# ingra14m/RobIR

Measured on AMD Instinct MI355X. Metric: PBR-stage rays/sec (128 SG lobes, 32 visibility samples/lobe), full forward render, higher is better.
Workload: dtype f32 (every MLP -- light visibility, SDF values and reverse-mode gradient, colour, visibility, 512-wide and CESR nets: every fp32 operand exact as three f16 pieces, six MFMA products per multiply-add in three fp32 accumulators -- in the light-visibility kernel the two outer products of the 2^-22 clas

## Files before the change

robir_amd/csrc/vis_diffuse_x6t.hip:

```cpp
#include "../../include/robir_hip.h"
#include "common.h"
#include "mlp_engine.h"
#include "x6_ring.h"

namespace rb {

#define RB_TINY 1e-6f
constexpr int XT_MAX_DIRS = 4096;
constexpr int XT_WF4 = 1536;
constexpr int XT_CF4 = 4 + XT_WF4;
constexpr int XT_SLOTS = 4, XT_DIST = 3;
constexpr int XT_PIECES = 6;
#ifndef XT_FP8
#define XT_FP8 1
#endif
template <int N>
struct XtInt {
  static constexpr int value = N;
};
__host__ __device__ constexpr bool xt_slot_tile0(int s) { return s == 0 || s == 1 || (s >= 4 && s <= 7); }

__device__ __forceinline__ void xt_dma16(const f4* gbase_uniform, unsigned lane_byte_off, unsigned lds_byte_uniform) {
  asm volatile("s_mov_b32 m0, %0\n\ts_nop 0\n\tglobal_load_lds_dwordx4 %1, %2" ::"s"(lds_byte_uniform), "v"(lane_byte_off),
               "s"(gbase_uniform)
               : "memory");
}
template <int OFF>
__device__ __forceinline__ void xt_dma16_imm(const f4* gbase_uniform, unsigned lane_byte_off, unsigned lds_byte_uniform) {
  asm volatile("s_mov_b32 m0, %0\n\ts_nop 0\n\tglobal_load_lds_dwordx4 %1, %2 offset:%3" ::"s"(lds_byte_uniform), "v"(lane_byte_off),
               "s"(gbase_uniform), "n"(OFF)
               : "memory");
}

template <int OFF>
__device__ __forceinline__ void xt_dma16_m0kept(const f4* gbase_uniform, unsigned lane_byte_off) {
  asm volatile("global_load_lds_dwordx4 %0, %1 offset:%2" ::"v"(lane_byte_off), "s"(gbase_uniform), "n"(OFF) : "memory");
}

struct XtTile {
  int point;
  int dir_base;
};
struct XtArgs {
  const float *A, *Bd;
  const f4* W49;
  int argmax_vis;
  unsigned* range_word;
  const float *normals, *dirs, *wdir, *wsum;
  const int* cid;
  int L, nsamp;
  float* vis_out;
  unsigned long long* eval_count;
  const unsigned short* pair_j;
  const XtTile* tile_info;
  const unsigned long long* counters;
  float* pair_vis;
};

template <bool STREAM>
__global__ __launch_bounds__(256, 1) void k_dvis_x6t(const XtArgs a) {
  __shared__ f4 ring[XT_SLOTS * XT_WF4];
  __shared__ f4 headw[XT_WF4];
  __shared__ f4 bias_tab[49 * 4];
  __shared__ f4 aux[(XT_MAX_DIRS * 4 + XT_MAX_DIRS * 2) / 16 + 64];
  __shared__ int s_count;
  float* const vis_tab = reinterpret_cast<float*>(aux);
  unsigned short* const idx_list = reinterpret_cast<unsigned short*>(aux + XT_MAX_DIRS / 4);
  f4* const a_row = aux + (XT_MAX_DIRS * 6) / 16;
  f4* const a_rows = aux;
  const float* __restrict__ A = a.A;
  const float* __restrict__ Bd = a.Bd;
  const f4* __restrict__ W49 = a.W49;
  const int argmax_vis = a.argmax_vis;
  const int tid = threadIdx.x, lane = tid & 63, g = lane >> 4;
  const int wave = __builtin_amdgcn_readfirstlane(tid >> 6);
  const float negk = -2048.0f;
  constexpr float C11 = 1.0f / 2048.0f;
  const long p = blockIdx.x;
  const int L = a.L, nsamp = a.nsamp, LS = L * nsamp;
  long dbase = 0;
  int S = 0, rounds = 0;
  const int G = gridDim.x;
  long total_tiles = 0, total_rounds = 0;
  for (int i = tid; i < 49 * 4; i += 256) bias_tab[i] = W49[(long)(i >> 2) * XT_CF4 + (i & 3)];
  for (int i = tid; i < XT_WF4; i += 256) headw[i] = W49[48L * XT_CF4 + 4 + i];
  if constexpr (STREAM) {
    total_tiles = (long)a.counters[0];
    total_rounds = (total_tiles + 7) >> 3;
    __syncthreads();
    if ((long)blockIdx.x >= total_rounds) return;
    rounds = 1;
  } else {
  const float* __restrict__ normals = a.normals;
  const float* __restrict__ dirs = a.dirs;
  const int* __restrict__ cid = a.cid;
  dbase = (cid ? (long)cid[p] : 0L) * LS;
  if (tid == 0) s_count = 0;
  if (tid < 64) a_row[tid] = reinterpret_cast<const f4*>(A + p * 256)[tid];
  for (int j = tid; j < LS; j += 256) vis_tab[j] = 0.f;
  __syncthreads();
  const float nx = normals[3 * p], ny = normals[3 * p + 1], nz = normals[3 * p + 2];
  for (int j0 = 0; j0 < LS; j0 += 256) {
    const int j = j0 + tid;
    bool front = false;
    if (j < LS) {
      const float* d = dirs + 3 * (dbase + j);
      const float c = nx * d[0] + ny * d[1] + nz * d[2];
      front = c > RB_TINY;
    }
    const unsigned long long mk = __ballot(front);
    int base = 0;
    if (lane == 0 && mk) base = atomicAdd(&s_count, __popcll(mk));
    base = __shfl(base, 0);
    if (front) idx_list[base + __popcll(mk & ((1ull << lane) - 1ull))] = (unsigned short)j;
  }
  __syncthreads();
  S = s_count;
  if (tid == 0 && a.eval_count) atomicAdd(a.eval_count, (unsigned long long)S);
  rounds = (S + 127) / 128;
  }

  const unsigned ring_b = (unsigned)(unsigned long)((__attribute__((address_space(3))) char*)ring);
  unsigned voff_a = (unsigned)wave * 6144u + (unsigned)lane * 16u, voff_b = voff_a + 4096u;
  asm volatile("" : "+v"(voff_a), "+v"(voff_b));
  const unsigned wave_lds = ring_b + (unsigned)wave * 6144u;
  typedef const __attribute__((address_space(3))) u4* lds_u4p;
  unsigned ring_a0 = ring_b + (unsigned)lane * 16u, ring_a2 = ring_a0 + 2u * XT_WF4 * 16u;
  asm volatile("" : "+v"(ring_a0), "+v"(ring_a2));
  const lds_u4p ring_u = (lds_u4p)ring_a0, ring_u2 = (lds_u4p)ring_a2;
  u4 wh[4], wm[4], wl[4];
#if XT_FP8
  typedef int xt_i8 __attribute__((ext_vector_type(8)));
  xt_i8 w8h, w8l;
#define XT_F16OFF(KB, PIECE) (((KB) >> 2) * 768 + (((KB) & 3) * 2 + (PIECE)) * 64)
#define XT_LOAD8(DST, BASE, OFF)                                                                                             \
  {                                                                                                                          \
    const u4 a_ = (BASE)[(OFF)], b_ = (BASE)[(OFF) + 64];                                                                    \
    DST = xt_i8{(int)a_[0], (int)a_[1], (int)a_[2], (int)a_[3], (int)b_[0], (int)b_[1], (int)b_[2], (int)b_[3]};             \
  }
#endif
  f4 bias;
  if (rounds > 0) {
#pragma unroll
    for (int c = 0; c < 3; ++c)
#pragma unroll
      for (int i = 0; i < XT_PIECES; ++i)
        xt_dma16(W49 + (long)c * XT_CF4 + 4 + i * 64, voff_a, wave_lds + (unsigned)c * 24576u + (unsigned)i * 1024u);
    asm volatile("s_waitcnt vmcnt(12)" ::: "memory");
    __builtin_amdgcn_s_barrier();
    asm volatile("" ::: "memory");
#pragma unroll
    for (int k = 0; k < 4; ++k) {
#if XT_FP8
      wh[k] = ring_u[XT_F16OFF(k, 0)];
      wm[k] = ring_u[XT_F16OFF(k, 1)];
#else
      wh[k] = ring_u[(k * 3 + 0) * 64];
      wm[k] = ring_u[(k * 3 + 1) * 64];
      wl[k] = ring_u[(k * 3 + 2) * 64];
#endif
    }
#if XT_FP8
    XT_LOAD8(w8h, ring_u, 512)
    XT_LOAD8(w8l, ring_u, 640)
#endif
    bias = bias_tab[g];
  }

  unsigned sat = 0u;
#if XT_FP8
  struct Ops {
    u4 h[2][8], m[2][8];
    xt_i8 h8[2][2], l8[2][2];
  };
  unsigned el_keep[2] = {0u, 0u};
#else
  struct Ops {
    u4 h[2][8], m[2][8], l[2][8];
  };
#endif
  Ops P, Q;

#define XT_MFMA(ACC, WREG, XREG) \
  ACC = __builtin_amdgcn_mfma_f32_16x16x32_f16(__builtin_bit_cast(h8, WREG), __builtin_bit_cast(h8, XREG), ACC, 0, 0, 0)

  float ev0[2][2], ev1[2][2], ed0, ed1;
  unsigned eh;
  SxAcc prev[2];
  auto ep_stage1 = [&](int t, int q) {
    const SxAcc& a = prev[t];
    const float r0 = __builtin_fmaf(__builtin_fmaf(a.c2[2 * q], C11, a.c1[2 * q]), C11, a.c0[2 * q]);
    const float r1 = __builtin_fmaf(__builtin_fmaf(a.c2[2 * q + 1], C11, a.c1[2 * q + 1]), C11, a.c0[2 * q + 1]);
    ev0[t][q] = fmaxf(r0, 0.f);
    ev1[t][q] = fmaxf(r1, 0.f);
  };
  auto ep_stage2 = [&](int t, int q) {
    const unsigned hu = __builtin_bit_cast(unsigned, __builtin_amdgcn_cvt_pkrtz(ev0[t][q], ev1[t][q]));
    const float s0 = ev0[t][q] * 2048.0f, s1 = ev1[t][q] * 2048.0f;
    asm("v_fma_mix_f32 %0, %1, %2, %3 op_sel_hi:[1,0,0]" : "=v"(ed0) : "v"(hu), "s"(negk), "v"(s0));
    asm("v_fma_mix_f32 %0, %1, %2, %3 op_sel:[1,0,0] op_sel_hi:[1,0,0]" : "=v"(ed1) : "v"(hu), "s"(negk), "v"(s1));
    eh = hu;
    sat = sat_acc_nonneg(sat, hu);
  };
  auto ep_stage3 = [&](Ops& Y, int t, int jb, int q) {
    const unsigned mu = __builtin_bit_cast(unsigned, __builtin_amdgcn_cvt_pkrtz(ed0, ed1));
    const float e0 = ed0 * 2048.0f, e1 = ed1 * 2048.0f;
    unsigned lu;
    asm("v_fma_mixlo_f16 %0, %1, %2, %3 op_sel_hi:[1,0,0]" : "=v"(lu) : "v"(mu), "s"(negk), "v"(e0));
    asm("v_fma_mixhi_f16 %0, %1, %2, %3 op_sel:[1,0,0] op_sel_hi:[1,0,0]" : "+v"(lu) : "v"(mu), "s"(negk), "v"(e1));
    Y.h[t][jb >> 1][(jb & 1) * 2 + q] = eh;
    Y.m[t][jb >> 1][(jb & 1) * 2 + q] = mu;
#if XT_FP8
    if (q == 0) {
      el_keep[t] = lu;
    } else {
      Y.h8[t][jb >> 3][jb & 7] = (int)__builtin_amdgcn_perm(eh, Y.h[t][jb >> 1][(jb & 1) * 2], 0x07050301u);
      Y.l8[t][jb >> 3][jb & 7] = (int)__builtin_amdgcn_perm(lu, el_keep[t], 0x07050301u);
    }
#else
    Y.l[t][jb >> 1][(jb & 1) * 2 + q] = lu;
#endif
  };
  auto ep_slot = [&](Ops& Y, int s, int pj) {
    switch (s) {
      case 0: ep_stage1(0, 0); break;
      case 1: ep_stage1(0, 1); break;
      case 2: ep_stage1(1, 0); break;
      case 3: ep_stage1(1, 1); break;
      case 4: ep_stage2(0, 0); break;
      case 5: ep_stage3(Y, 0, pj, 0); break;
      case 6: ep_stage2(0, 1); break;
      case 7: ep_stage3(Y, 0, pj, 1); break;
      case 8: ep_stage2(1, 0); break;
      case 9: ep_stage3(Y, 1, pj, 0); break;
      case 10: ep_stage2(1, 1); break;
      default: ep_stage3(Y, 1, pj, 1); break;
    }
  };

  f4 raw[2][16];
  int jj[2], jjn[2];
  int tpn[2] = {-1, -1}, tbn[2] = {0, 0}, jn2[2] = {0xFFFF, 0xFFFF};
  const unsigned arow_b = (unsigned)(unsigned long)((__attribute__((address_space(3))) char*)a_rows);
  XtTile recn[2] = {{-1, 0}, {-1, 0}};
  bool okn[2] = {false, false};
  auto tile_lookup = [&](long round) {
#pragma unroll
    for (int t = 0; t < 2; ++t) {
      const long T = round * 8 + wave * 2 + t;
      okn[t] = round < total_rounds && T < total_tiles;
      const long Tc = T < total_tiles ? T : total_tiles - 1;
      recn[t] = a.tile_info[Tc];
      jn2[t] = (int)a.pair_j[Tc * 16 + (lane & 15)];
    }
  };
  auto tile_resolve = [&]() {
#pragma unroll
    for (int t = 0; t < 2; ++t) {
      tpn[t] = okn[t] ? __builtin_amdgcn_readfirstlane(recn[t].point) : -1;
      tbn[t] = okn[t] ? __builtin_amdgcn_readfirstlane(recn[t].dir_base) : 0;
      if (!okn[t]) jn2[t] = 0xFFFF;
    }
  };
  auto fetch_rows = [&](long rd_next, int parity_next) {
    if constexpr (STREAM) {
      tile_resolve();
#pragma unroll
      for (int t = 0; t < 2; ++t) {
        const long prow = tpn[t] < 0 ? 0L : (long)tpn[t];
        xt_dma16(reinterpret_cast<const f4*>(A + prow * 256), (unsigned)lane * 16u,
                 arow_b + (unsigned)(parity_next * 8 + wave * 2 + t) * 1024u);
      }
    }
#pragma unroll
    for (int t = 0; t < 2; ++t) {
      long row;
      if constexpr (STREAM) {
        jjn[t] = (tpn[t] < 0 || jn2[t] == 0xFFFF) ? -1 : jn2[t];
        row = (long)tbn[t] + (jjn[t] < 0 ? 0 : jjn[t]);
      } else {
        const int si = (int)rd_next * 128 + t * 64 + wave * 16 + (lane & 15);
        jjn[t] = si < S ? (int)idx_list[si] : -1;
        row = dbase + (jjn[t] < 0 ? 0 : jjn[t]);
      }
      const f4* brow = reinterpret_cast<const f4*>(Bd + row * 256) + g;
#pragma unroll
      for (int kb = 0; kb < 16; ++kb) raw[t][kb] = brow[kb * 4];
    }
  };
  long rd = STREAM ? (long)blockIdx.x : 0L;
  const long rd_end = STREAM ? total_rounds : (long)rounds, rd_step = STREAM ? (long)G : 1L;
  int parity = 0;
  if constexpr (STREAM) tile_lookup(rd);
  if (rounds > 0) fetch_rows(rd, 0);
#ifdef XT_TIMING
#define XT_T(i) { const unsigned long long t_ = __builtin_amdgcn_s_memtime(); tacc[i] += t_ - tlast; tlast = t_; }
  unsigned long long tacc[4] = {0, 0, 0, 0}, tlast = __builtin_amdgcn_s_memtime();
  int trounds = 0;
#else
#define XT_T(i)
#endif
  {
    auto round_body = [&](auto ntc) __attribute__((always_inline)) {
    constexpr int NT = decltype(ntc)::value;
#pragma unroll
    for (int t = 0; t < NT; ++t) {
      jj[t] = jjn[t];
      const f4* arow = STREAM ? a_rows + (parity * 8 + wave * 2 + t) * 64 : a_row;
#pragma unroll
      for (int kb = 0; kb < 16; ++kb) {
        const f4 bv = raw[t][kb];
        const f4 av = arow[kb * 4 + g];
#pragma unroll
        for (int q = 0; q < 2; ++q) {
          unsigned h, m, l;
          sx_split_pair(fmaxf(av[2 * q] + bv[2 * q], 0.f), fmaxf(av[2 * q + 1] + bv[2 * q + 1], 0.f), negk, h, m, l);
          P.h[t][kb / 2][(kb & 1) * 2 + q] = h;
          P.m[t][kb / 2][(kb & 1) * 2 + q] = m;
#if XT_FP8
          if (q == 0) {
            el_keep[t] = l;
          } else {
            P.h8[t][kb >> 3][kb & 7] = (int)__builtin_amdgcn_perm(h, P.h[t][kb / 2][(kb & 1) * 2], 0x07050301u);
            P.l8[t][kb >> 3][kb & 7] = (int)__builtin_amdgcn_perm(l, el_keep[t], 0x07050301u);
          }
#else
          P.l[t][kb / 2][(kb & 1) * 2 + q] = l;
#endif
          sat = sat_acc_nonneg(sat, h);
        }
      }
    }
    XT_T(0)
    auto layer = [&](int l, Ops& X, Ops& Y) __attribute__((always_inline)) {
      const f4* Wl = W49 + (long)l * 16 * XT_CF4 + 4;
      const f4* Wn = W49 + (long)(l == 2 ? 0 : l + 1) * 16 * XT_CF4 + 4;
#pragma unroll
      for (int jb = 0; jb < 16; ++jb) {
        SxAcc acc[2];
        asm volatile("s_waitcnt vmcnt(6)" ::: "memory");
#ifndef XT_ABL_NOBAR
        __builtin_amdgcn_s_barrier();
#endif
        asm volatile("" ::: "memory");
        const int nx3 = jb + XT_DIST;
        const f4* dsrc = nx3 < 16 ? Wl + (long)nx3 * XT_CF4 : Wn + (long)(nx3 - 16) * XT_CF4;
        const unsigned ddst = wave_lds + (unsigned)(nx3 & 3) * 24576u;
        const f4 nbias = bias_tab[(l * 16 + jb + 1) * 4 + g];
#if defined(XT_ABL_NODMA)
#define XT_COPY(I) do { } while (0)
#else
#define XT_COPY(I)                                                                  \
  do {                                                                              \
    if ((I) == 0) xt_dma16_imm<0>(dsrc, voff_a, ddst);                              \
    else if ((I) < 4) xt_dma16_m0kept<((I) & 3) * 1024>(dsrc, voff_a);              \
    else if ((I) == 4) xt_dma16_imm<0>(dsrc, voff_b, ddst + 4096u);                 \
    else xt_dma16_m0kept<((I) & 3) * 1024>(dsrc, voff_b);                           \
  } while (0)
#endif
#define XT_FENCE __builtin_amdgcn_sched_barrier(0)
#ifdef XT_ABL_NOLDS
#define XT_FRAG(DST, KB, PIECE) asm volatile("" : "+v"(DST))
#else
#if XT_FP8
#define XT_FRAG(DST, KB, PIECE) DST = nfrag[XT_F16OFF(KB, PIECE)]
#else
#define XT_FRAG(DST, KB, PIECE) DST = nfrag[((KB) * 3 + (PIECE)) * 64]
#endif
#endif
#define XT_MFMA8(ACC, WREG, XREG) ACC = __builtin_amdgcn_mfma_scale_f32_16x16x128_f8f6f4(WREG, XREG, ACC, 1, 1, 0, 0, 0, 0)
#define XT_EP(S)                        \
  do {                                  \
    if (jb > 0) ep_slot(Y, (S), jb - 1); \
  } while (0)
#define XT_RUN(ACC, WP, XP)                     \
  _Pragma("unroll") for (int k_ = 0; k_ < 4; ++k_) { \
    const int k = H ? 3 - k_ : k_;               \
    XT_MFMA(ACC, WP[k], XP[4 * H + k]);          \
  }
#define XT_RUN_REFILL(ACC, WP, XP, PIECE)          \
  _Pragma("unroll") for (int k_ = 0; k_ < 4; ++k_) { \
    const int k = H ? 3 - k_ : k_;                   \
    XT_MFMA(ACC, WP[k], XP[4 * H + k]);              \
// ... 128 lines not shown
#if !XT_FP8
          P.l[t][kb] = Q.l[t][kb];
#endif
        }
#if XT_FP8
#pragma unroll
      for (int t = 0; t < NT; ++t)
#pragma unroll
        for (int hf = 0; hf < 2; ++hf) {
          P.h8[t][hf] = Q.h8[t][hf];
          P.l8[t][hf] = Q.l8[t][hf];
        }
#endif
    }
    XT_T(1)
    if constexpr (STREAM) fetch_rows(rd + rd_step, parity ^ 1);
    else if constexpr (NT == 2) fetch_rows(rd + 1 < rd_end ? rd + 1 : rd, 0);
    {
      const u4* hw = reinterpret_cast<const u4*>(headw) + lane;
      SxAcc acc[2];
#pragma unroll
      for (int t = 0; t < NT; ++t) {
        acc[t].c0 = bias;
        acc[t].c1 = f4{0.f, 0.f, 0.f, 0.f};
        acc[t].c2 = f4{0.f, 0.f, 0.f, 0.f};
      }
#pragma unroll
#if XT_FP8
      for (int kb = 0; kb < 8; ++kb) {
        const u4 fh = hw[XT_F16OFF(kb, 0)], fm = hw[XT_F16OFF(kb, 1)];
#pragma unroll
        for (int t = 0; t < NT; ++t) {
          XT_MFMA(acc[t].c0, fh, P.h[t][kb]);
          XT_MFMA(acc[t].c1, fh, P.m[t][kb]);
          XT_MFMA(acc[t].c1, fm, P.h[t][kb]);
          XT_MFMA(acc[t].c2, fm, P.m[t][kb]);
        }
      }
#pragma unroll
      for (int hf = 0; hf < 2; ++hf) {
        xt_i8 f8h, f8l;
        XT_LOAD8(f8h, hw, hf * 768 + 512)
        XT_LOAD8(f8l, hw, hf * 768 + 640)
#pragma unroll
        for (int t = 0; t < NT; ++t) {
          acc[t].c2 = __builtin_amdgcn_mfma_scale_f32_16x16x128_f8f6f4(f8h, P.l8[t][hf], acc[t].c2, 1, 1, 0, 0, 0, 0);
          acc[t].c2 = __builtin_amdgcn_mfma_scale_f32_16x16x128_f8f6f4(f8l, P.h8[t][hf], acc[t].c2, 1, 1, 0, 0, 0, 0);
        }
      }
#else
      for (int kb = 0; kb < 8; ++kb) {
        const u4 fh = hw[(kb * 3 + 0) * 64], fm = hw[(kb * 3 + 1) * 64], fl = hw[(kb * 3 + 2) * 64];
#pragma unroll
        for (int t = 0; t < NT; ++t) {
          XT_MFMA(acc[t].c0, fh, P.h[t][kb]);
          XT_MFMA(acc[t].c1, fh, P.m[t][kb]);
          XT_MFMA(acc[t].c2, fh, P.l[t][kb]);
          XT_MFMA(acc[t].c1, fm, P.h[t][kb]);
          XT_MFMA(acc[t].c2, fm, P.m[t][kb]);
          XT_MFMA(acc[t].c2, fl, P.h[t][kb]);
        }
      }
#endif
      bias = bias_tab[g];
#pragma unroll
      for (int t = 0; t < NT; ++t) {
        const float l0 = __builtin_fmaf(__builtin_fmaf(acc[t].c2[0], C11, acc[t].c1[0]), C11, acc[t].c0[0]);
        const float l1 = __builtin_fmaf(__builtin_fmaf(acc[t].c2[1], C11, acc[t].c1[1]), C11, acc[t].c0[1]);
        if (g == 0 && jj[t] >= 0) {
          float v;
          if (argmax_vis) {
            v = l1 > l0 ? 1.f : 0.f;
          } else {
            const float mx = fmaxf(l0, l1);
            const float e0 = expf(l0 - mx), e1 = expf(l1 - mx);
            v = e1 / (e0 + e1);
          }
          if constexpr (STREAM) a.pair_vis[(rd * 8 + wave * 2 + t) * 16 + (lane & 15)] = v;
          else vis_tab[jj[t]] = v;
        }
      }
    }
    };
    const bool tail1 = !STREAM && XT_FP8 && rounds > 0 && S - (rounds - 1) * 128 <= 64;
    const long rd_end2 = tail1 ? rd_end - 1 : rd_end;
    for (; rd < rd_end2; rd += rd_step) {
      if constexpr (STREAM) tile_lookup(rd + rd_step);
#ifdef XT_TIMING
      ++trounds;
#endif
      XT_T(3)
      round_body(XtInt<2>{});
      parity ^= 1;
      XT_T(2)
    }
    if constexpr (!STREAM && XT_FP8) {
      if (tail1) {
#ifdef XT_TIMING
        ++trounds;
#endif
        XT_T(3)
        round_body(XtInt<1>{});
        XT_T(2)
      }
    }
  }
#ifdef XT_TIMING
  if ((blockIdx.x == 7 || blockIdx.x == 4000) && tid == 0 && trounds > 0)
    printf("x6t wg %d rounds %d cycles/round: conv %llu layers %llu head+fetch %llu lookup %llu\n", (int)blockIdx.x, trounds, tacc[0] / trounds,
           tacc[1] / trounds, tacc[2] / trounds, tacc[3] / trounds);
#endif
#undef XT_MFMA
  range_report<true>(sat, a.range_word);
  asm volatile("s_waitcnt vmcnt(0)" ::: "memory");
  __syncthreads();
  if constexpr (!STREAM) {
    if (tid < L) {
      const float* w = a.wdir + dbase + (long)tid * nsamp;
      float acc = 0.f;
      for (int k = 0; k < nsamp; ++k) acc += vis_tab[tid * nsamp + k] * w[k];
      a.vis_out[p * L + tid] = acc / a.wsum[(a.cid ? a.cid[p] : 0) * L + tid];
    }
  }
}

struct V3Tile;
__global__ void k_dvis3_cull(const float* __restrict__ normals, const int* __restrict__ cid, long n, const float* __restrict__ dirs, int LS,
                             unsigned short* __restrict__ pair_j, V3Tile* __restrict__ tile_info, int2* __restrict__ point_info,
                             unsigned long long* __restrict__ counters, unsigned long long* __restrict__ eval_count);
__global__ void k_dvis3_reduce(const int* __restrict__ cid, long n, const float* __restrict__ wdir, const float* __restrict__ wsum,
                               const unsigned short* __restrict__ pair_j, const float* __restrict__ pair_vis,
                               const int2* __restrict__ point_info, int L, int nsamp, float* __restrict__ vis_out);

}

using namespace rb;

extern "C" int rb_dvis_fused_x6t(const float* normals, const int* chunk_id, long n, const float* A, const float* Bd,
                                 const float* dirs, const float* wdir, const float* wsum, const float* W49, int L, int nsamp,
                                 int argmax_vis, int scale_log2, float* vis_out, unsigned long long* eval_count,
                                 rb_stream_t stream) {
  if (n <= 0) return 0;
  RB_REQUIRE(normals && A && Bd && dirs && wdir && wsum && W49 && vis_out, "null pointer");
  RB_REQUIRE(n <= RB_MAX_BLOCKS, "too many points for one launch (one workgroup each)");
  RB_REQUIRE(L > 0 && L <= 256 && nsamp > 0 && (long)L * nsamp <= XT_MAX_DIRS, "need L <= 256 and L*nsamp <= 4096");
#if XT_FP8
  RB_REQUIRE(scale_log2 == 8, "this build of k_dvis_x6t takes the bf8 weight layout (packing.repack_x6_chunks_fp8; scale_log2 = 8 names it)");
#else
  RB_REQUIRE(scale_log2 == 0, "k_dvis_x6t takes weights packed with scale_log2 = 0");
#endif
  XtArgs a{};
  a.A = A, a.Bd = Bd, a.W49 = (const f4*)W49, a.argmax_vis = argmax_vis;
  a.range_word = range_flags() ? range_flags() + RB_RANGE_DVIS : nullptr;
  a.normals = normals, a.dirs = dirs, a.wdir = wdir, a.wsum = wsum, a.cid = chunk_id, a.L = L, a.nsamp = nsamp;
  a.vis_out = vis_out, a.eval_count = eval_count;
  hipLaunchKernelGGL(k_dvis_x6t<false>, dim3((unsigned)n), dim3(256), 0, (hipStream_t)stream, a);
  return check_launch("k_dvis_x6t");
}

extern "C" int rb_dvis_stream_x6(const float* normals, const int* chunk_id, long n, const float* A, const float* Bd,
                                 const float* dirs, const float* wdir, const float* wsum, const float* W49, int L, int nsamp,
                                 int argmax_vis, int scale_log2, unsigned short* pair_j, float* pair_vis, int* tile_info,
                                 int* point_info, unsigned long long* counters, int n_workgroups, float* vis_out,
                                 unsigned long long* eval_count, rb_stream_t stream) {
  if (n <= 0) return 0;
  RB_REQUIRE(normals && A && Bd && dirs && wdir && wsum && W49 && vis_out, "null pointer");
  RB_REQUIRE(pair_j && pair_vis && tile_info && point_info && counters, "null scratch pointer");
  RB_REQUIRE(n <= RB_MAX_BLOCKS, "too many points for one launch (one workgroup each in the cull / reduce passes)");
  RB_REQUIRE(L > 0 && L <= 256 && nsamp > 0 && (long)L * nsamp <= XT_MAX_DIRS && (L * nsamp) % 16 == 0,
             "need L <= 256, L*nsamp <= 4096 and a multiple of 16");
  RB_REQUIRE((long)n * (L * nsamp / 16) < (1L << 31), "tile index would overflow 31 bits");
#if XT_FP8
  RB_REQUIRE(scale_log2 == 8, "this build of k_dvis_x6t takes the bf8 weight layout (packing.repack_x6_chunks_fp8; scale_log2 = 8 names it)");
#else
  RB_REQUIRE(scale_log2 == 0, "k_dvis_x6t takes weights packed with scale_log2 = 0");
#endif
  hipStream_t s = (hipStream_t)stream;
  if (n_workgroups <= 0) n_workgroups = device_cus();
  RB_REQUIRE(n_workgroups > 0, "device query failed");
  if (hipMemsetAsync(counters, 0, 2 * sizeof(unsigned long long), s) != hipSuccess) return rb::fail(__func__, "memset failed");
  hipLaunchKernelGGL(k_dvis3_cull, dim3((unsigned)n), dim3(256), 0, s, normals, chunk_id, n, dirs, L * nsamp, pair_j,
                     reinterpret_cast<V3Tile*>(tile_info), reinterpret_cast<int2*>(point_info), counters, eval_count);
  if (int rc = check_launch("k_dvis3_cull")) return rc;
  XtArgs a{};
  a.A = A, a.Bd = Bd, a.W49 = (const f4*)W49, a.argmax_vis = argmax_vis;
  a.range_word = range_flags() ? range_flags() + RB_RANGE_DVIS : nullptr;
  a.pair_j = pair_j, a.tile_info = reinterpret_cast<const XtTile*>(tile_info), a.counters = counters, a.pair_vis = pair_vis;
  hipLaunchKernelGGL(k_dvis_x6t<true>, dim3((unsigned)n_workgroups), dim3(256), 0, s, a);
  if (int rc = check_launch("k_dvis_x6t<stream>")) return rc;
  hipLaunchKernelGGL(k_dvis3_reduce, dim3((unsigned)n), dim3(256), 0, s, chunk_id, n, wdir, wsum, pair_j, pair_vis,
                     reinterpret_cast<const int2*>(point_info), L, nsamp, vis_out);
  return check_launch("k_dvis3_reduce");
}
```

robir_amd/ops.py:

```python
import ctypes
import functools
import os

import torch

from . import _lib, dispatch
from ._lib import ptr, stream_ptr, call

c_long, c_int, c_float = ctypes.c_long, ctypes.c_int, ctypes.c_float


def _f32(t):
    assert t.dtype == torch.float32, t.dtype
    return t.contiguous()


RANGE_FAMILIES = ("light-visibility kernel (rb_dvis_fused*)", "visibility MLP (rb_vis_mlp_h3 / rb_vis_x6_points)",
                  "SDF MLP (rb_sdf_mlp_h3 / rb_sdf_x6_points / rb_sdf_value_grad*)", "colour MLP (rb_color_mlp_h3 / rb_color_x6_points)",
                  "512-wide nets (rb_wide_mlp_h3 / rb_wide_x6*)", "CESR nets (rb_cesr_net_h3 / rb_cesr_net_x6_points)")


def range_check(sync=False):
    mask = ctypes.c_uint(0)
    call("rb_range_check", c_int(1 if sync else 0), stream_ptr(), ctypes.byref(mask))
# ... 475 lines not shown
        n_layers=5, slab_rows=slab_rows, part_rows=part_rows, defaults=(ILLUM_SLAB_ROWS, ILLUM_PART_ROWS),
        launch=lambda P, G, tail: _lib.call_illumtrain("rb_it_lobe_bwd", ptr(points), ptr(hdr), c_long(n), P, ptr(g_sgs), G, *tail))


CESR_PARAM_NAMES = tuple(f"lin{l}.{w}" for l in range(9) for w in ("weight_g", "weight_v", "bias"))
CESR_KINDS = {"normal": (0, 63, 3), "shadow": (1, 191, 2)}
CESR_SLAB_ROWS = 16384
CESR_PART_ROWS = 1024


def cesr_backward(x, M, kind, params, g_out, head=0, n_label=1, want=CESR_PARAM_NAMES, slab_rows=None, part_rows=None):
    code, d_in, d_out = CESR_KINDS[kind]
    x = _f32(x.detach())
    M, dev = int(M), x.device
    points = x.dim() == 2 and x.shape[1] == 3
    assert x.dim() == 2 and len(params) == 27 and n_label >= 1 and M % n_label == 0
    assert (x.shape[0] * n_label == M) if points else (x.shape[0] == M and x.shape[1] >= d_in), "points [M / n_label, 3] or rows [M, >= d_in]"
    params = [_f32(p.detach()) for p in params]
    assert tuple(params[1].shape) == (512, d_in) and tuple(params[25].shape) == (d_out, 512), f"not the {kind} network's tensors"
    g_out = _f32(g_out.detach()).reshape((M,) if head == 1 else (M, d_out))
    return _partitioned_backward(
        "cesr_backward", CESR_PARAM_NAMES, params, want, rows=M, dev=dev, lib=_lib.cesrtrain, query="rb_ct_cesr_bwd_scratch_bytes", n_layers=9,
        slab_rows=slab_rows, part_rows=part_rows, defaults=(CESR_SLAB_ROWS, CESR_PART_ROWS),
        launch=lambda P, G, tail: _lib.call_cesrtrain(
            "rb_ct_cesr_bwd", ptr(x if points else None), ptr(None if points else x), c_long(x.shape[1]), c_long(M), c_int(code),
            c_int(n_label), c_int(head), P, ptr(g_out), G, *tail))


def _sg_query_args(sgs, dirs):
    sgs, dirs = _f32(sgs.detach()), _f32(dirs.detach())
    assert sgs.dim() == 3 and sgs.shape[2] == 7 and dirs.dim() == 3 and dirs.shape[2] == 3 and dirs.shape[0] == sgs.shape[0]
    return sgs, dirs, sgs.shape[0], sgs.shape[1], dirs.shape[1]


def sg_query(sgs, dirs):
    sgs, dirs, n, L, S = _sg_query_args(sgs, dirs)
    rad = torch.empty(n, S, 3, dtype=torch.float32, device=sgs.device)
    _lib.call_illumtrain("rb_it_sg_query", ptr(sgs), ptr(dirs), c_long(n), c_int(L), c_long(S), ptr(rad), stream_ptr())
    return rad


def sg_query_backward(sgs, dirs, g):
    sgs, dirs, n, L, S = _sg_query_args(sgs, dirs)
    g = _f32(g.detach()).reshape(n, S, 3)
    out = torch.empty(n, L, 7, dtype=torch.float32, device=sgs.device)
    _lib.call_illumtrain("rb_it_sg_query_bwd", ptr(sgs), ptr(dirs), ptr(g), c_long(n), c_int(L), c_long(S), ptr(out), stream_ptr())
    return out


def axpy(a, b, s):
    a, b = _f32(a), _f32(b)
    y = torch.empty_like(a)
    call("rb_axpy", ptr(a), ptr(b), c_float(s), c_long(a.numel()), ptr(y), stream_ptr())
    return y


def normalize3(x, eps, mode):
    x = _f32(x)
    y = torch.empty_like(x)
    call("rb_normalize3", ptr(x), c_long(x.shape[0]), c_float(eps), c_int(mode), ptr(y), stream_ptr())
    return y


def dvis_dirs(lgt, u_theta, u_phi, thr=1.0, direct=False):
    lgt, u_theta, u_phi = _f32(lgt), _f32(u_theta), _f32(u_phi)
    if u_theta.dim() == 2:
        u_theta, u_phi = u_theta[None], u_phi[None]
    C, L, ns = u_theta.shape
    dev = lgt.device
    dirs = torch.empty(C * L * ns, 3, dtype=torch.float32, device=dev)
    wdir = torch.empty(C * L * ns, dtype=torch.float32, device=dev)
    wsum = torch.empty(C * L, dtype=torch.float32, device=dev)
    call("rb_dvis_dirs", ptr(lgt), c_int(L), c_int(ns), c_int(C), c_int(1 if direct else 0), ptr(u_theta.contiguous()), ptr(u_phi.contiguous()),
         c_float(thr), ptr(dirs), ptr(wdir), ptr(wsum), stream_ptr())
    return dirs, wdir, wsum


DVIS_KERNEL_NAMES = {"fp32": "k_dvis_fused<fp32>", "f16x6": "k_dvis_x6t", "f16x6-pt": "k_dvis_x6t", "f16x6-stream": "k_dvis_x6t<stream>",
                     "f16x6-1t": "k_dvis_x6", "f16x1": "k_dvis_f16p", "f16x3-auto": "k_dvis_v2", "f16x3-v3": "k_dvis3_stream",
                     "f16x3-v2": "k_dvis_v2", "f16x3": "k_dvis_fused<H3>"}


DVIS_STREAM_WORKGROUPS = 0
DVIS_STREAM_MAX_POINTS = 8192
DVIS_STREAM_SHORT_LIST = 1024
DVIS_F16_GEN = int(os.environ.get("ROBIR_DVIS_F16_GEN", "3"))


def chunk_ids_ascending(chunk_id):
    if chunk_id is None or chunk_id.numel() < 2:
        return True
    known = getattr(chunk_id, "_robir_ascending", None)
    if known is None:
        known = bool((chunk_id[1:] >= chunk_id[:-1]).all())
        chunk_id._robir_ascending = known
    return known
DVIS_X6_FP8 = os.environ.get("ROBIR_DVIS_X6_FP8", "1") == "1"
DVIS_X6_FORM = os.environ.get("ROBIR_DVIS_X6_FORM", "auto")


def dvis_fused(normals, chunk_id, A, Bd, dirs, wdir, wsum, split, L, nsamp, argmax_vis=False, eval_count=None,
               precision="fp32"):
    normals = _f32(normals)
    n, dev = normals.shape[0], normals.device
    r = dispatch.dvis(precision, n, L, nsamp, DVIS_X6_FORM, DVIS_X6_FP8, DVIS_F16_GEN, lambda: chunk_ids_ascending(chunk_id),
                      DVIS_STREAM_MAX_POINTS, DVIS_STREAM_SHORT_LIST)
    out = torch.empty(n, L, dtype=torch.float32, device=dev)
    if chunk_id is not None:
        assert chunk_id.dtype == torch.int32
    args = [ptr(normals), ptr(chunk_id), c_long(n), ptr(A), ptr(Bd), ptr(dirs), ptr(wdir), ptr(wsum), ptr(split[r.blob])]
    if r.layout == "gen1":
        args += [ptr(split["w_last"]), ptr(split["b_last"])]
    args += [c_int(L), c_int(nsamp), c_int(1 if argmax_vis else 0)]
    if r.layout == "gen1":
        args.append(c_int(5 if r.legacy else 0))
    if r.fmt is not None:
        args.append(c_int(split[r.fmt] if isinstance(r.fmt, str) else r.fmt))
    LS = L * nsamp
    if r.layout == "pblock":
        items_max = (n + 15) // 16 + max(1, dirs.shape[0] // LS) - 1
        entries = torch.empty(items_max * LS, dtype=torch.int32, device=dev)
        pair_vis = torch.empty(items_max * LS * 16, dtype=torch.float32, device=dev)
        round_info = torch.empty(items_max * LS // 16, 4, dtype=torch.int32, device=dev)
        item_info = torch.empty(items_max, 4, dtype=torch.int32, device=dev)
        counters = torch.empty(4, dtype=torch.int64, device=dev)
        args += [c_int(items_max), ptr(entries), ptr(pair_vis), ptr(round_info), ptr(item_info), ptr(counters), c_int(DVIS_STREAM_WORKGROUPS)]
    elif r.layout == "stream":
        pair_j = torch.empty(n * LS, dtype=torch.int16, device=dev)
        pair_vis = torch.empty(n * LS, dtype=torch.float32, device=dev)
        tile_info = torch.empty(n * LS // 16, 2, dtype=torch.int32, device=dev)
        point_info = torch.empty(n, 2, dtype=torch.int32, device=dev)
        counters = torch.empty(2, dtype=torch.int64, device=dev)
        args += [ptr(pair_j), ptr(pair_vis), ptr(tile_info), ptr(point_info), ptr(counters), c_int(DVIS_STREAM_WORKGROUPS)]
    (_lib.call_legacy if r.legacy else call)(r.entry, *args, ptr(out), ptr(eval_count), stream_ptr())
    if r.layout == "pblock" and os.environ.get("ROBIR_RANGE_CHECK", "") == "sync" and int(counters[3].item()) != 0:
        raise _lib.RobirHipError("rb_dvis_pblock_f16: chunk ids are not ascending or the item scratch overflowed -- the outputs "
                                 "of this call are NaN (ADVICE r5; run without the `_robir_ascending` tag to let ops check the order)")
    return out


def _spec_vis_buffers(n, ns, n_chunks, dev):
    return (torch.empty(n, dtype=torch.float32, device=dev), torch.empty(n_chunks, dtype=torch.int32, device=dev),
            torch.empty(n * ns, 3, dtype=torch.float32, device=dev), torch.empty(n * ns, dtype=torch.float32, device=dev),
            torch.empty(n * ns, dtype=torch.uint8, device=dev))


def spec_vis_sample(normal, view, rough, chunk_id, n_chunks, u_theta, u_phi):
    normal, view, rough = _f32(normal), _f32(view), _f32(rough).reshape(-1)
    u_theta, u_phi = _f32(u_theta), _f32(u_phi)
    n, ns = u_theta.shape
    sharp, cmin, dirs, wts, front = _spec_vis_buffers(n, ns, n_chunks, normal.device)
    call("rb_spec_vis_sample", ptr(normal), ptr(view), ptr(rough), ptr(chunk_id), c_long(n), c_int(n_chunks), c_int(ns),
         ptr(u_theta), ptr(u_phi), ptr(sharp), ptr(cmin), ptr(dirs), ptr(wts), ptr(front), stream_ptr())
    return dirs, wts, front


def spec_vis_sample_lobes(normal, view, lobes, lambdas, chunk_id, n_chunks, u_theta, u_phi):
    normal, view, lobes, lambdas = _f32(normal), _f32(view), _f32(lobes), _f32(lambdas).reshape(-1)
    u_theta, u_phi = _f32(u_theta), _f32(u_phi)
    n, ns = u_theta.shape
    assert lobes.shape == (n, 3) and lambdas.shape == (n,), (lobes.shape, lambdas.shape)
    sharp, cmin, dirs, wts, front = _spec_vis_buffers(n, ns, n_chunks, normal.device)
    call("rb_spec_vis_sample_lobes", ptr(normal), ptr(view), ptr(lobes), ptr(lambdas), ptr(chunk_id), c_long(n), c_int(n_chunks), c_int(ns),
         ptr(u_theta), ptr(u_phi), ptr(sharp), ptr(cmin), ptr(dirs), ptr(wts), ptr(front), stream_ptr())
    return dirs, wts, front


def spec_vis_reduce(logits, front, wts, n, nsamp, inv, argmax_vis, testing):
    bvis = torch.empty(n, dtype=torch.float32, device=logits.device)
    call("rb_spec_vis_reduce", ptr(logits), ptr(front), ptr(wts), c_long(n), c_int(nsamp), c_int(int(inv)),
         c_int(int(argmax_vis)), c_int(int(testing)), ptr(bvis), stream_ptr())
    return bvis


def _f0_tensor(f0, dev):
    if isinstance(f0, torch.Tensor):
        return f0.detach().to(device=dev, dtype=torch.float32).reshape(-1)[:1].contiguous()
    return torch.full((1,), float(f0), device=dev)


def sg_shade(normal, view, lgt, f0, rough, albedo, bvis, light_vis=None, metallic=None, indir_integral=None,
             lin_diff=False, want_shadow=False):
    normal, view, lgt, albedo = _f32(normal), _f32(view), _f32(lgt), _f32(albedo)
    rough = _f32(rough).reshape(-1)
    n = normal.shape[0]
    per_point = lgt.dim() == 3
    M = lgt.shape[-2]
    dev = normal.device
    rgb, spec, diff = (torch.empty(n, 3, dtype=torch.float32, device=dev) for _ in range(3))
    shadow = torch.empty(n, 3, dtype=torch.float32, device=dev) if want_shadow else None
    f0 = _f0_tensor(f0, dev)
    call("rb_sg_shade", ptr(normal), ptr(view), ptr(lgt), c_int(1 if per_point else 0), c_int(M), ptr(f0), ptr(rough),
         ptr(albedo), ptr(_f32(metallic).reshape(-1) if metallic is not None else None),
         ptr(_f32(light_vis) if light_vis is not None else None), ptr(bvis),
         ptr(_f32(indir_integral) if indir_integral is not None else None), c_int(1 if lin_diff else 0), c_long(n),
         ptr(rgb), ptr(spec), ptr(diff), ptr(shadow), stream_ptr())
    return rgb, spec, diff, shadow


def sg_shade_backward(normal, view, lgt, f0, rough, albedo, bvis, spec, diff, g_spec, g_diff, light_vis=None, metallic=None,
                      indir_integral=None, lin_diff=False, want=("lgt", "f0", "rough", "albedo", "metallic", "bvis", "light_vis", "indir_integral")):
    normal, view, lgt, albedo = _f32(normal), _f32(view), _f32(lgt), _f32(albedo)
    rough, bvis = _f32(rough).reshape(-1), _f32(bvis).reshape(-1)
    spec, diff, g_spec, g_diff = _f32(spec), _f32(diff), _f32(g_spec), _f32(g_diff)
    n = normal.shape[0]
    per_point = lgt.dim() == 3
    M = lgt.shape[-2]
    dev = normal.device
    f0 = _f0_tensor(f0, dev)
    metallic = _f32(metallic).reshape(-1) if metallic is not None else None
    light_vis = _f32(light_vis) if light_vis is not None else None
    indir_integral = _f32(indir_integral) if indir_integral is not None else None
    shapes = {"lgt": tuple(lgt.shape), "f0": (1,), "rough": (n,), "albedo": (n, 3), "bvis": (n,)}
    if metallic is not None:
        shapes["metallic"] = (n,)
    if light_vis is not None:
# ... 601 lines not shown
```

Measured before the change: 512,700.

## Make per-point diffuse visibility kernel persistent with an atomic point queue

```diff
diff --git a/robir_amd/csrc/vis_diffuse_x6t.hip b/robir_amd/csrc/vis_diffuse_x6t.hip
--- a/robir_amd/csrc/vis_diffuse_x6t.hip
+++ b/robir_amd/csrc/vis_diffuse_x6t.hip
@@ -2,6 +2,9 @@
 #include "common.h"
 #include "mlp_engine.h"
 #include "x6_ring.h"
+#include <atomic>
+#include <cstdlib>
+#include <mutex>
 
 namespace rb {
 
@@ -51,6 +54,8 @@
   int L, nsamp;
   float* vis_out;
   unsigned long long* eval_count;
+  long n;
+  unsigned* queue;
   const unsigned short* pair_j;
   const XtTile* tile_info;
   const unsigned long long* counters;
@@ -64,6 +69,7 @@
   __shared__ f4 bias_tab[49 * 4];
   __shared__ f4 aux[(XT_MAX_DIRS * 4 + XT_MAX_DIRS * 2) / 16 + 64];
   __shared__ int s_count;
+  __shared__ unsigned s_next;
   float* const vis_tab = reinterpret_cast<float*>(aux);
   unsigned short* const idx_list = reinterpret_cast<unsigned short*>(aux + XT_MAX_DIRS / 4);
   f4* const a_row = aux + (XT_MAX_DIRS * 6) / 16;
@@ -76,10 +82,11 @@
   const int wave = __builtin_amdgcn_readfirstlane(tid >> 6);
   const float negk = -2048.0f;
   constexpr float C11 = 1.0f / 2048.0f;
-  const long p = blockIdx.x;
+  long p = 0;
   const int L = a.L, nsamp = a.nsamp, LS = L * nsamp;
   long dbase = 0;
   int S = 0, rounds = 0;
+  unsigned long long evals = 0;
   const int G = gridDim.x;
   long total_tiles = 0, total_rounds = 0;
   for (int i = tid; i < 49 * 4; i += 256) bias_tab[i] = W49[(long)(i >> 2) * XT_CF4 + (i & 3)];
@@ -91,33 +98,7 @@
     if ((long)blockIdx.x >= total_rounds) return;
     rounds = 1;
   } else {
-  const float* __restrict__ normals = a.normals;
-  const float* __restrict__ dirs = a.dirs;
-  const int* __restrict__ cid = a.cid;
-  dbase = (cid ? (long)cid[p] : 0L) * LS;
-  if (tid == 0) s_count = 0;
-  if (tid < 64) a_row[tid] = reinterpret_cast<const f4*>(A + p * 256)[tid];
-  for (int j = tid; j < LS; j += 256) vis_tab[j] = 0.f;
-  __syncthreads();
-  const float nx = normals[3 * p], ny = normals[3 * p + 1], nz = normals[3 * p + 2];
-  for (int j0 = 0; j0 < LS; j0 += 256) {
-    const int j = j0 + tid;
-    bool front = false;
-    if (j < LS) {
-      const float* d = dirs + 3 * (dbase + j);
-      const float c = nx * d[0] + ny * d[1] + nz * d[2];
-      front = c > RB_TINY;
-    }
-    const unsigned long long mk = __ballot(front);
-    int base = 0;
-    if (lane == 0 && mk) base = atomicAdd(&s_count, __popcll(mk));
-    base = __shfl(base, 0);
-    if (front) idx_list[base + __popcll(mk & ((1ull << lane) - 1ull))] = (unsigned short)j;
-  }
-  __syncthreads();
-  S = s_count;
-  if (tid == 0 && a.eval_count) atomicAdd(a.eval_count, (unsigned long long)S);
-  rounds = (S + 127) / 128;
+    __syncthreads();
   }
 
   const unsigned ring_b = (unsigned)(unsigned long)((__attribute__((address_space(3))) char*)ring);
@@ -140,7 +121,7 @@
   }
 #endif
   f4 bias;
-  if (rounds > 0) {
+  if (!STREAM || rounds > 0) {
 #pragma unroll
     for (int c = 0; c < 3; ++c)
 #pragma unroll
@@ -288,17 +269,77 @@
       for (int kb = 0; kb < 16; ++kb) raw[t][kb] = brow[kb * 4];
     }
   };
+  auto point_begin = [&]() -> bool {
+    int btid = tid;
+    asm volatile("" : "+v"(btid));
+    const int blane = btid & 63;
+    const float* __restrict__ normals = a.normals;
+    const float* __restrict__ dirs = a.dirs;
+    const int* __restrict__ cid = a.cid;
+    if (btid == 0) {
+      s_next = atomicAdd(a.queue, 1u);
+      s_count = 0;
+    }
+    __syncthreads();
+    const long pn = (long)(unsigned)__builtin_amdgcn_readfirstlane((int)s_next);
+    if (pn >= a.n) return false;
+    p = pn;
+    dbase = (cid ? (long)cid[p] : 0L) * LS;
+    if (btid < 64) a_row[btid] = reinterpret_cast<const f4*>(A + p * 256)[btid];
+    for (int j = btid; j < LS; j += 256) vis_tab[j] = 0.f;
+    const float nx = normals[3 * p], ny = normals[3 * p + 1], nz = normals[3 * p + 2];
+    for (int j0 = 0; j0 < LS; j0 += 256) {
+      const int j = j0 + btid;
+      bool front = false;
+      if (j < LS) {
+        const float* d = dirs + 3 * (dbase + j);
+        const float c = nx * d[0] + ny * d[1] + nz * d[2];
+        front = c > RB_TINY;
+      }
+      const unsigned long long mk = __ballot(front);
+      int base = 0;
+      if (blane == 0 && mk) base = atomicAdd(&s_count, __popcll(mk));
+      base = __shfl(base, 0);
+      if (front) idx_list[base + __popcll(mk & ((1ull << blane) - 1ull))] = (unsigned short)j;
+    }
+    asm volatile("s_waitcnt vmcnt(0)" ::: "memory");
+    __syncthreads();
+    S = __builtin_amdgcn_readfirstlane(s_count);
+    evals += (unsigned long long)S;
+    rounds = (S + 127) / 128;
+    if (rounds > 0) fetch_rows(0, 0);
+    return true;
+  };
+  auto point_end = [&]() {
+    int btid = tid;
+    asm volatile("" : "+v"(btid));
+    __syncthreads();
+    if (btid < L) {
+      const float* w = a.wdir + dbase + (long)btid * nsamp;
+      float acc = 0.f;
+      for (int k = 0; k < nsamp; ++k) acc += vis_tab[btid * nsamp + k] * w[k];
+      a.vis_out[p * L + btid] = acc / a.wsum[(a.cid ? a.cid[p] : 0) * L + btid];
+    }
+  };
   long rd = STREAM ? (long)blockIdx.x : 0L;
-  const long rd_end = STREAM ? total_rounds : (long)rounds, rd_step = STREAM ? (long)G : 1L;
+  long rd_end = STREAM ? total_rounds : 0L;
+  const long rd_step = STREAM ? (long)G : 1L;
   int parity = 0;
-  if constexpr (STREAM) tile_lookup(rd);
-  if (rounds > 0) fetch_rows(rd, 0);
+  if constexpr (STREAM) {
+    tile_lookup(rd);
+    fetch_rows(rd, 0);
+  }
 #ifdef XT_TIMING
 #define XT_T(i) { const unsigned long long t_ = __builtin_amdgcn_s_memtime(); tacc[i] += t_ - tlast; tlast = t_; }
   unsigned long long tacc[4] = {0, 0, 0, 0}, tlast = __builtin_amdgcn_s_memtime();
   int trounds = 0;
+#define XT_PT(i) { const unsigned long long t_ = __builtin_amdgcn_s_memrealtime(); ptacc[i] += t_ - ptlast; ptlast = t_; }
+  unsigned long long ptacc[3] = {0, 0, 0}, ptlast = __builtin_amdgcn_s_memrealtime();
+  const unsigned long long pt_first = ptlast;
+  int tpoints = 0;
 #else
 #define XT_T(i)
+#define XT_PT(i)
 #endif
   {
     auto round_body = [&](auto ntc) __attribute__((always_inline)) {
@@ -593,46 +634,59 @@
       }
     }
     };
-    const bool tail1 = !STREAM && XT_FP8 && rounds > 0 && S - (rounds - 1) * 128 <= 64;
-    const long rd_end2 = tail1 ? rd_end - 1 : rd_end;
-    for (; rd < rd_end2; rd += rd_step) {
-      if constexpr (STREAM) tile_lookup(rd + rd_step);
+    for (;;) {
+      if constexpr (!STREAM) {
+        if (!point_begin()) break;
+        rd = 0, rd_end = (long)rounds;
 #ifdef XT_TIMING
-      ++trounds;
-#endif
-      XT_T(3)
-      round_body(XtInt<2>{});
-      parity ^= 1;
-      XT_T(2)
-    }
-    if constexpr (!STREAM && XT_FP8) {
-      if (tail1) {
+        ++tpoints;
+        tlast = __builtin_amdgcn_s_memtime();
+#endif
+        XT_PT(0)
+      }
+      const bool tail1 = !STREAM && XT_FP8 && rounds > 0 && S - (rounds - 1) * 128 <= 64;
+      const long rd_end2 = tail1 ? rd_end - 1 : rd_end;
+      for (; rd < rd_end2; rd += rd_step) {
+        if constexpr (STREAM) tile_lookup(rd + rd_step);
 #ifdef XT_TIMING
         ++trounds;
 #endif
         XT_T(3)
-        round_body(XtInt<1>{});
+        round_body(XtInt<2>{});
+        parity ^= 1;
         XT_T(2)
       }
-    }
-  }
+      if constexpr (!STREAM && XT_FP8) {
+        if (tail1) {
 #ifdef XT_TIMING
-  if ((blockIdx.x == 7 || blockIdx.x == 4000) && tid == 0 && trounds > 0)
+          ++trounds;
+#endif
+          XT_T(3)
+          round_body(XtInt<1>{});
+          XT_T(2)
+        }
+      }
+      if constexpr (STREAM) break;
+      XT_PT(1)
+      point_end();
+      XT_PT(2)
+    }
+  }
+#ifdef XT_TIMING
+  if ((STREAM ? blockIdx.x == 7 || blockIdx.x == 4000 : (blockIdx.x & 31) == 7) && tid == 0 && trounds > 0)
     printf("x6t wg %d rounds %d cycles/round: conv %llu layers %llu head+fetch %llu lookup %llu\n", (int)blockIdx.x, trounds, tacc[0] / trounds,
            tacc[1] / trounds, tacc[2] / trounds, tacc[3] / trounds);
+  if (!STREAM && (blockIdx.x & 31) == 7 && tid == 0 && tpoints > 0)
+    printf("x6t wg %d points %d rounds %d ticks(10 ns) in all: boundary %llu rounds %llu reduce %llu workgroup %llu\n", (int)blockIdx.x, tpoints,
+           trounds, ptacc[0], ptacc[1], ptacc[2], __builtin_amdgcn_s_memrealtime() - pt_first);
 #endif
 #undef XT_MFMA
   range_report<true>(sat, a.range_word);
+  if constexpr (!STREAM) {
+    if (tid == 0 && a.eval_count) atomicAdd(a.eval_count, evals);
+  }
   asm volatile("s_waitcnt vmcnt(0)" ::: "memory");
   __syncthreads();
-  if constexpr (!STREAM) {
-    if (tid < L) {
-      const float* w = a.wdir + dbase + (long)tid * nsamp;
-      float acc = 0.f;
-      for (int k = 0; k < nsamp; ++k) acc += vis_tab[tid * nsamp + k] * w[k];
-      a.vis_out[p * L + tid] = acc / a.wsum[(a.cid ? a.cid[p] : 0) * L + tid];
-    }
-  }
 }
 
 struct V3Tile;
@@ -646,6 +700,31 @@
 }
 
 using namespace rb;
+
+constexpr int XT_QUEUES = 256, XT_MAX_DEVICES = 64;
+static unsigned* g_pt_queues[XT_MAX_DEVICES] = {};
+static std::atomic<unsigned> g_pt_turn{0};
+static std::mutex g_pt_mutex;
+static unsigned* pt_queue() {
+  int dev = 0;
+  if (hipGetDevice(&dev) != hipSuccess || dev < 0 || dev >= XT_MAX_DEVICES) return nullptr;
+  std::lock_guard<std::mutex> lock(g_pt_mutex);
+  if (!g_pt_queues[dev]) {
+    void* d = nullptr;
+    if (hipMalloc(&d, XT_QUEUES * sizeof(unsigned)) != hipSuccess) {
+      (void)hipGetLastError();
+      return nullptr;
+    }
+    g_pt_queues[dev] = static_cast<unsigned*>(d);
+  }
+  return g_pt_queues[dev] + g_pt_turn.fetch_add(1u) % XT_QUEUES;
+}
+
+static int pt_workgroups() {
+  const char* e = getenv("ROBIR_DVIS_PT_WORKGROUPS");
+  const int w = e ? atoi(e) : 0;
+  return w > 0 ? w : 0;
+}
 
 extern "C" int rb_dvis_fused_x6t(const float* normals, const int* chunk_id, long n, const float* A, const float* Bd,
                                  const float* dirs, const float* wdir, const float* wsum, const float* W49, int L, int nsamp,
@@ -665,7 +744,12 @@
   a.range_word = range_flags() ? range_flags() + RB_RANGE_DVIS : nullptr;
   a.normals = normals, a.dirs = dirs, a.wdir = wdir, a.wsum = wsum, a.cid = chunk_id, a.L = L, a.nsamp = nsamp;
   a.vis_out = vis_out, a.eval_count = eval_count;
-  hipLaunchKernelGGL(k_dvis_x6t<false>, dim3((unsigned)n), dim3(256), 0, (hipStream_t)stream, a);
+  const int grid = persistent_grid(n, pt_workgroups());
+  RB_REQUIRE(grid > 0, "device query failed");
+  a.n = n, a.queue = pt_queue();
+  RB_REQUIRE(a.queue, "no device memory for the point queue");
+  if (hipMemsetAsync(a.queue, 0, sizeof(unsigned), (hipStream_t)stream) != hipSuccess) return rb::fail(__func__, "memset failed");
+  hipLaunchKernelGGL(k_dvis_x6t<false>, dim3((unsigned)grid), dim3(256), 0, (hipStream_t)stream, a);
   return check_launch("k_dvis_x6t");
 }
 
diff --git a/robir_amd/ops.py b/robir_amd/ops.py
--- a/robir_amd/ops.py
+++ b/robir_amd/ops.py
@@ -581,6 +581,8 @@
 
 
 DVIS_STREAM_WORKGROUPS = 0
+DVIS_PT_WORKGROUPS = int(os.environ.get("ROBIR_DVIS_PT_WORKGROUPS") or 0)
+_dvis_pt_workgroups_env = DVIS_PT_WORKGROUPS
 DVIS_STREAM_MAX_POINTS = 8192
 DVIS_STREAM_SHORT_LIST = 1024
 DVIS_F16_GEN = int(os.environ.get("ROBIR_DVIS_F16_GEN", "3"))
@@ -631,6 +633,11 @@
         point_info = torch.empty(n, 2, dtype=torch.int32, device=dev)
         counters = torch.empty(2, dtype=torch.int64, device=dev)
         args += [ptr(pair_j), ptr(pair_vis), ptr(tile_info), ptr(point_info), ptr(counters), c_int(DVIS_STREAM_WORKGROUPS)]
+    elif r.entry == "rb_dvis_fused_x6t":
+        global _dvis_pt_workgroups_env
+        if int(DVIS_PT_WORKGROUPS) != _dvis_pt_workgroups_env:
+            _dvis_pt_workgroups_env = int(DVIS_PT_WORKGROUPS)
+            os.environ["ROBIR_DVIS_PT_WORKGROUPS"] = str(max(0, _dvis_pt_workgroups_env))
     (_lib.call_legacy if r.legacy else call)(r.entry, *args, ptr(out), ptr(eval_count), stream_ptr())
     if r.layout == "pblock" and os.environ.get("ROBIR_RANGE_CHECK", "") == "sync" and int(counters[3].item()) != 0:
         raise _lib.RobirHipError("rb_dvis_pblock_f16: chunk ids are not ascending or the item scratch overflowed -- the outputs "
```

After: 524,100, median of 6. 1.02x the previous value.
